# SamuelCancilla2/radar-point-cloud-tracking

Hardware: NVIDIA B200
Metric: fused_frames_per_s_through_stdbscan (higher is better)
Workload: dtype f32 (points) / f64 (neighbour test) / i32 (labels)

## Files before the change

### radar_point_cloud_tracking_b200/csrc/common.cuh

```cuda
#pragma once
#include <cuda_runtime.h>
#include <stdint.h>
#include <stdio.h>
#include <string.h>

#include <utility>
#include <vector>

#include "radarb200.h"

#define RB_WARP 32

struct rb_scratch {
    void* ptr = nullptr;
    size_t cap = 0;
};

enum rb_slot {
    RB_S_TILE_STATUS = 0,
    RB_S_SWEEP_FLAGS,
    RB_S_SPOKE_MASK,
    RB_S_REDUCE,
    RB_S_KEEP,
    RB_S_BLOCKSUM,
    RB_S_BLOCKSUM2,
    RB_S_CELL_ID,
    RB_S_CELL_START,
    RB_S_CELL_FILL,
    RB_S_SORT_IDX,
    RB_S_SX, RB_S_SY, RB_S_SZ, RB_S_ST,
    RB_S_CORE,
    RB_S_PARENT,
    RB_S_MINORIG,
    RB_S_FLAGS,
    RB_S_RANK,
    RB_S_SLABEL,
    RB_S_STATS,
    RB_S_MISC,
    RB_S_FUSE_GRID,
    RB_S_COMP_KEY,
    RB_S_PIPE, RB_S_PIPE_EDGES, RB_S_PIPE_TIMES,
    RB_S_B_NCORE, RB_S_B_PARENT, RB_S_B_LABEL, RB_S_B_MINKEY, RB_S_CORE_START, RB_S_CB_LIST,
    RB_S_CSV,
    RB_S_CLUSTERS,
    RB_S_LAND_FLAG,
    RB_S_SHARD_IDS, RB_S_SHARD_LOCAL, RB_S_SHARD_KEYS,
    RB_S_GROUP_TMP,
    RB_S_LAND_ORDERED,
    RB_S_REC_FRAMES,
    RB_S_REC_LOCAL,
    RB_S_REC_KEYS,
    RB_S_REC_KEYS_BIG,
    RB_S_REC_TABLE,
    RB_S_REC_CORE,
    RB_S_COUNT
};

struct rb_db_plan;
struct rb_comm;

struct rb_ctx {
    int device = 0;
    int sm_count = 0;
    int cc_major = 0, cc_minor = 0;
    int64_t l2_bytes = 0;
    int64_t launches = 0;
    rb_scratch slots[RB_S_COUNT];
    std::vector<void*> retired;
    void* pinned = nullptr;
    size_t pinned_cap = 0;
    rb_dbscan_stats last_stats;
    rb_db_plan* db_plan = nullptr;
    rb_comm* comm = nullptr;
    int64_t rec_key_cap = 0;
    int opt_dbscan_mode = 0;
    int opt_spoke_mask_variant = 0;
    int spoke_last_variant = 0;
    int opt_spoke_profile = 0;
    int opt_spoke_ring = 2;
    int opt_spoke_l2_hint = 1;
    int opt_mask_priority = 1;
    int prio_high = 0;
    int opt_mask_gate = 1;
    int opt_carveout = -1;
    unsigned attr_spoke_mask = 0;
    bool attr_land = false;
    cudaEvent_t spoke_ev[4] = {nullptr, nullptr, nullptr, nullptr};
};

void rb_set_error(const char* fmt, ...);
void rb_db_plan_free(rb_ctx* ctx);
void rb_comm_free(rb_ctx* ctx);
int rb_scratch_get(rb_ctx* ctx, rb_slot slot, size_t bytes, void** out);

#define RB_CUDA(call)                                                                      \
    do {                                                                                   \
        cudaError_t _e = (call);                                                           \
        if (_e != cudaSuccess) {                                                           \
            rb_set_error("%s:%d: %s -> %s", __FILE__, __LINE__, #call, cudaGetErrorString(_e)); \
            return RB_ERR_CUDA;                                                            \
        }                                                                                  \
    } while (0)

#define RB_LAUNCH_CHECK(ctx)                                                               \
    do {                                                                                   \
        (ctx)->launches++;                                                                 \
        cudaError_t _e = cudaGetLastError();                                               \
        if (_e != cudaSuccess) {                                                           \
            rb_set_error("%s:%d: kernel launch -> %s", __FILE__, __LINE__, cudaGetErrorString(_e)); \
            return RB_ERR_CUDA;                                                            \
        }                                                                                  \
    } while (0)

#define RB_REQUIRE(cond, msg)                                                              \
    do {                                                                                   \
        if (!(cond)) {                                                                     \
            rb_set_error("%s:%d: %s", __FILE__, __LINE__, msg);                            \
            return RB_ERR_ARG;                                                             \
        }                                                                                  \
    } while (0)

#define RB_TRY(expr)                                                                       \
    do {                                                                                   \
        int _rc = (expr);                                                                  \
        if (_rc != RB_OK) return _rc;                                                      \
    } while (0)

static inline int64_t rb_div_up(int64_t a, int64_t b) { return (a + b - 1) / b; }
// ... 82 lines not shown
```

### radar_point_cloud_tracking_b200/csrc/context.cu

```cuda
#include <stdarg.h>
#include <stdlib.h>

#include "common.cuh"

static thread_local char g_err[512] = "";

void rb_set_error(const char* fmt, ...) {
    va_list ap;
    va_start(ap, fmt);
    vsnprintf(g_err, sizeof g_err, fmt, ap);
    va_end(ap);
}

extern "C" const char* rb_last_error(void) { return g_err; }
extern "C" int rb_version(void) { return 1; }

extern "C" int rb_create(int device, rb_ctx** out) {
    if (!out) { rb_set_error("rb_create: out is NULL"); return RB_ERR_ARG; }
    *out = nullptr;
    int n = 0;
    cudaError_t e = cudaGetDeviceCount(&n);
    if (e != cudaSuccess || n <= 0) {
        rb_set_error("rb_create: no CUDA device (%s); this library has no CPU fallback",
                     e == cudaSuccess ? "device count 0" : cudaGetErrorString(e));
        return RB_ERR_CUDA;
    }
    if (device < 0 || device >= n) { rb_set_error("rb_create: bad device %d of %d", device, n); return RB_ERR_ARG; }
    int prev = -1;
    RB_CUDA(cudaGetDevice(&prev));
    struct Restore { int d; ~Restore() { if (d >= 0) cudaSetDevice(d); } } restore{prev == device ? -1 : prev};
    RB_CUDA(cudaSetDevice(device));
    cudaDeviceProp prop;
    RB_CUDA(cudaGetDeviceProperties(&prop, device));
    if (prop.major < 10) {
        rb_set_error("rb_create: device %d is sm_%d%d; this build is sm_100a only", device, prop.major, prop.minor);
        return RB_ERR_CUDA;
    }
    rb_ctx* ctx = new rb_ctx();
    ctx->device = device;
    ctx->sm_count = prop.multiProcessorCount;
    ctx->cc_major = prop.major;
    ctx->cc_minor = prop.minor;
    ctx->l2_bytes = prop.l2CacheSize;
    int prio_low = 0, prio_high = 0;
    if (cudaDeviceGetStreamPriorityRange(&prio_low, &prio_high) == cudaSuccess) ctx->prio_high = prio_high;
    memset(&ctx->last_stats, 0, sizeof ctx->last_stats);
    ctx->pinned_cap = 1 << 20;
    e = cudaMallocHost(&ctx->pinned, ctx->pinned_cap);
    if (e != cudaSuccess) {
        rb_set_error("rb_create: cudaMallocHost -> %s", cudaGetErrorString(e));
        delete ctx;
        return RB_ERR_NOMEM;
    }
    static const char* const env_opts[] = {"carveout", "spoke_ring", "spoke_l2_hint", "dbscan_mode", "spoke_mask_variant", "mask_gate", "mask_priority"};
    for (const char* name : env_opts) {
        char var[64] = "RB_OPT_";
        size_t k = strlen(var);
        for (const char* c = name; *c && k + 1 < sizeof var; ++c) var[k++] = (char)(*c >= 'a' && *c <= 'z' ? *c - 32 : *c);
        var[k] = 0;
        const char* v = getenv(var);
        if (v && *v && rb_set_option(ctx, name, atoll(v)) != RB_OK) { rb_destroy(ctx); return RB_ERR_ARG; }
    }
    *out = ctx;
    return RB_OK;
}

extern "C" void rb_destroy(rb_ctx* ctx) {
    if (!ctx) return;
    cudaSetDevice(ctx->device);
    for (int i = 0; i < RB_S_COUNT; ++i)
        if (ctx->slots[i].ptr) cudaFree(ctx->slots[i].ptr);
    for (void* p : ctx->retired) cudaFree(p);
    if (ctx->pinned) cudaFreeHost(ctx->pinned);
    for (int i = 0; i < 4; ++i)
        if (ctx->spoke_ev[i]) cudaEventDestroy(ctx->spoke_ev[i]);
    rb_db_plan_free(ctx);
    rb_comm_free(ctx);
    delete ctx;
}

extern "C" int rb_device_info(rb_ctx* ctx, int* sm_count, int* cc_major, int* cc_minor, int64_t* l2_bytes) {
    RB_REQUIRE(ctx, "ctx is NULL");
    if (sm_count) *sm_count = ctx->sm_count;
    if (cc_major) *cc_major = ctx->cc_major;
    if (cc_minor) *cc_minor = ctx->cc_minor;
    if (l2_bytes) *l2_bytes = ctx->l2_bytes;
    return RB_OK;
}

extern "C" int rb_set_option(rb_ctx* ctx, const char* name, int64_t value) {
    RB_REQUIRE(ctx && name, "NULL argument");
    if (!strcmp(name, "spoke_profile")) { ctx->opt_spoke_profile = value != 0; return RB_OK; }
    if (!strcmp(name, "dbscan_mode")) {
        RB_REQUIRE(value >= 0 && value <= 2, "dbscan_mode: 0 = auto, 1 = general algorithm, 2 = require the tight-cell algorithm");
        ctx->opt_dbscan_mode = (int)value;
        return RB_OK;
    }
    if (!strcmp(name, "spoke_mask_variant")) {
        RB_REQUIRE(value >= 0 && value <= 2, "spoke_mask_variant: 0 = auto, 1 = register-staged, 2 = TMA-staged");
        ctx->opt_spoke_mask_variant = (int)value;
        return RB_OK;
    }
    if (!strcmp(name, "spoke_ring")) {
        RB_REQUIRE(value >= 0 && value <= 3, "spoke_ring: 0 = 64 KiB x 3, 1 = 32 KiB x 4, 2 = 32 KiB x 3 (default), 3 = 48 KiB x 2");
        ctx->opt_spoke_ring = (int)value;
        return RB_OK;
    }
    if (!strcmp(name, "spoke_l2_hint")) { ctx->opt_spoke_l2_hint = value != 0; return RB_OK; }
    if (!strcmp(name, "mask_gate")) { ctx->opt_mask_gate = value != 0; return RB_OK; }
    if (!strcmp(name, "mask_priority")) { ctx->opt_mask_priority = value != 0; return RB_OK; }
    if (!strcmp(name, "carveout")) {
        RB_REQUIRE(value >= -1 && value <= 100, "carveout: -1 = the driver's choice per kernel, 0..100 = percent of the SM's shared memory");
        ctx->opt_carveout = (int)value;
        return RB_OK;
    }
    rb_set_error("rb_set_option: unknown option '%s'", name);
    return RB_ERR_ARG;
}

extern "C" int64_t rb_get_info(rb_ctx* ctx, const char* name) {
    if (!ctx || !name) return -1;
    if (!strcmp(name, "launches")) return ctx->launches;
    if (!strcmp(name, "spoke_profile")) return ctx->opt_spoke_profile;
    if (!strcmp(name, "spoke_mask_variant")) return ctx->opt_spoke_mask_variant;
    if (!strcmp(name, "dbscan_mode")) return ctx->opt_dbscan_mode;
    if (!strcmp(name, "spoke_last_variant")) return ctx->spoke_last_variant;
    if (!strcmp(name, "spoke_ring")) return ctx->opt_spoke_ring;
    if (!strcmp(name, "spoke_l2_hint")) return ctx->opt_spoke_l2_hint;
    if (!strcmp(name, "mask_gate")) return ctx->opt_mask_gate;
    if (!strcmp(name, "mask_priority")) return ctx->opt_mask_priority;
    if (!strcmp(name, "carveout")) return ctx->opt_carveout;
    int k = !strcmp(name, "spoke_mask_ns") ? 0 : !strcmp(name, "spoke_offsets_ns") ? 1 : !strcmp(name, "spoke_emit_ns") ? 2 : -1;
    if (k >= 0) {
        if (!ctx->spoke_ev[3]) return -1;
        if (cudaEventSynchronize(ctx->spoke_ev[3]) != cudaSuccess) return -1;
        float ms = 0.f;
        if (cudaEventElapsedTime(&ms, ctx->spoke_ev[k], ctx->spoke_ev[k + 1]) != cudaSuccess) return -1;
        return (int64_t)((double)ms * 1e6);
    }
    return -1;
}

extern "C" int64_t rb_launch_count(rb_ctx* ctx) { return ctx ? ctx->launches : -1; }

extern "C" int rb_trim(rb_ctx* ctx) {
    RB_REQUIRE(ctx, "ctx is NULL");
    for (void* p : ctx->retired) cudaFree(p);
    ctx->retired.clear();
    return RB_OK;
}

int rb_scratch_get(rb_ctx* ctx, rb_slot slot, size_t bytes, void** out) {
    rb_scratch& s = ctx->slots[slot];
    if (bytes == 0) bytes = 16;
    if (s.cap < bytes) {
        if (s.ptr) {
            ctx->retired.push_back(s.ptr);
            s.ptr = nullptr;
            s.cap = 0;
        }
        size_t want = bytes + bytes / 2;
        want = (want + 255) & ~size_t(255);
        cudaError_t e = cudaMalloc(&s.ptr, want);
        if (e != cudaSuccess) {
            rb_set_error("scratch slot %d: cudaMalloc(%zu) -> %s", (int)slot, want, cudaGetErrorString(e));
            s.ptr = nullptr;
            return RB_ERR_NOMEM;
        }
        s.cap = want;
    }
    *out = s.ptr;
    return RB_OK;
}

constexpr int SCAN_THREADS = 256;
constexpr int SCAN_ITEMS = 8;
constexpr int SCAN_TILE = SCAN_THREADS * SCAN_ITEMS;

// ... 102 lines not shown
```

### radar_point_cloud_tracking_b200/csrc/dbscan.cu

```cuda
#include <float.h>
#include <math.h>

#include "common.cuh"

namespace {

constexpr int DB_THREADS = 256;
constexpr long long KEY_NONE = 0x7fffffffffffffffLL;

struct DbGrid {
    double lo[3];
    double inv_cell;
    double tmin;
    double inv_wt;
    int n[3];
    int nt;
    int tr;
    int dim;
    int R;
    int tight;
};

struct DbPoints {
    const float* x; const float* y; const float* z;
// ... 299 lines not shown
__global__ void __launch_bounds__(DB_THREADS) dbg_keyout_kernel(int n, const uint8_t* __restrict__ core, const int* __restrict__ parent,
                                                               const int* __restrict__ sidx, const long long* __restrict__ minkey,
                                                               long long* __restrict__ comp_key) {
    int p = blockIdx.x * blockDim.x + threadIdx.x;
    if (p >= n) return;
    comp_key[sidx[p]] = core[p] == 1 ? minkey[parent[p]] : -1;
}

template <int DIM, bool WF>
__global__ void __launch_bounds__(DB_THREADS) dbg_border_kernel(Sorted s, DbGrid g, double eps2, float eps_t,
                                                               const uint8_t* __restrict__ core, const int* __restrict__ slabel,
                                                               const int* __restrict__ sidx, const long long* __restrict__ comp_key,
                                                               const int* __restrict__ open_list, const int* __restrict__ n_open,
                                                               int32_t* __restrict__ labels, unsigned long long* __restrict__ ctr) {
    const int total = *n_open;
    unsigned long long tests = 0;
    for (int i = blockIdx.x * blockDim.x + threadIdx.x; i < total; i += gridDim.x * blockDim.x) {
        const int p = open_list[i];
        Pt<DIM> a = load_pt<DIM>(s, p);
        int best = INT_MAX;
        for_each_candidate<DIM>(g, s.cell_start, s.cell[p], [&](int q) {
            if (core[q] == 1) {
                int lq = slabel[q];
                if (lq < best) {
                    if (WF) {
                        const int oq = sidx[q];
                        const long long start = comp_key[oq];
                        if (!(start < (long long)sidx[p] || start == (long long)oq)) return true;
                    }
                    ++tests;
                    if (is_neighbour<DIM>(a, load_pt<DIM>(s, q), eps2, eps_t)) best = lq;
                }
            }
            return best != 0;
        });
        if (best != INT_MAX) labels[sidx[p]] = best;
    }
    add_counter(ctr, tests);
}

struct Window {
    int x0, x1, y0, y1, z0, z1, t0, t1;
};
template <int DIM>
__device__ __forceinline__ Window window_of(const DbGrid& g, const CellPos& c) {
    Window w;
    w.x0 = max(c.cx - g.R, 0); w.x1 = min(c.cx + g.R, g.n[0] - 1);
    w.y0 = DIM > 1 ? max(c.cy - g.R, 0) : 0; w.y1 = DIM > 1 ? min(c.cy + g.R, g.n[1] - 1) : 0;
    w.z0 = DIM > 2 ? max(c.cz - g.R, 0) : 0; w.z1 = DIM > 2 ? min(c.cz + g.R, g.n[2] - 1) : 0;
    w.t0 = max(c.tb - g.tr, 0); w.t1 = min(c.tb + g.tr, g.nt - 1);
    return w;
}

template <int DIM, bool WF>
__global__ void __launch_bounds__(DB_THREADS) dbt_count_kernel(Sorted s, DbGrid g, int n, double eps2, int min_samples, int min_frames,
                                                              uint8_t* __restrict__ core, unsigned long long* __restrict__ ctr) {
    int p = blockIdx.x * blockDim.x + threadIdx.x;
    unsigned long long tests = 0;
    if (p < n) {
        const int cell = s.cell[p];
        const CellPos c = decode_cell(g, cell);
        const Window w = window_of<DIM>(g, c);
        const int per_t = g.n[0] * g.n[1] * g.n[2];
        const int sp = cell - c.tb * per_t;
        int cnt = 0;
        unsigned long long frames = 0;
        for (int tt = w.t0; tt <= w.t1; ++tt) {
            const int k = s.cell_start[tt * per_t + sp + 1] - s.cell_start[tt * per_t + sp];
            cnt += k;
            if (WF && k > 0) frames |= 1ull << (tt - w.t0);
        }
        auto open = [&]() { return cnt < min_samples || (WF && __popcll(frames) < min_frames); };
        if (open()) {
            const Pt<DIM> a = load_pt<DIM>(s, p);
            for (int tt = w.t0; tt <= w.t1 && open(); ++tt)
                for (int zz = w.z0; zz <= w.z1 && open(); ++zz)
                    for (int yy = w.y0; yy <= w.y1 && open(); ++yy) {
                        const int row = ((tt * g.n[2] + zz) * g.n[1] + yy) * g.n[0];
                        const bool own_row = zz == c.cz && yy == c.cy;
                        const int b = s.cell_start[row + w.x0], e = s.cell_start[row + w.x1 + 1];
                        int hb = e, he = e;
                        if (own_row) { hb = s.cell_start[row + c.cx]; he = s.cell_start[row + c.cx + 1]; }
                        for (int q = b; q < hb && open(); ++q) {
                            ++tests;
                            if (near_enough<DIM>(a, load_pt<DIM>(s, q), eps2)) { ++cnt; if (WF) frames |= 1ull << (tt - w.t0); }
                        }
                        for (int q = he; q < e && open(); ++q) {
                            ++tests;
                            if (near_enough<DIM>(a, load_pt<DIM>(s, q), eps2)) { ++cnt; if (WF) frames |= 1ull << (tt - w.t0); }
                        }
                    }
        }
        core[p] = !open() ? 1 : (cnt <= 1 ? 2 : 0);
    }
    add_counter(ctr, tests);
}

__global__ void __launch_bounds__(DB_THREADS) dbt_bucket_init_kernel(int64_t n_cells, int* __restrict__ b_ncore, int* __restrict__ b_parent,
                                                                    long long* __restrict__ b_minkey, int* __restrict__ n_cb) {
    int64_t b = (int64_t)blockIdx.x * blockDim.x + threadIdx.x;
    if (b == 0) *n_cb = 0;
    if (b < n_cells) { b_ncore[b] = 0; b_minkey[b] = KEY_NONE; }
    if (b == n_cells) b_ncore[b] = 0;
}

template <typename T, typename Op>
__device__ __forceinline__ T seg_reduce_sorted(T v, int key, Op op) {
    const unsigned lane = rb_lane();
#pragma unroll
    for (int d = 1; d < 32; d <<= 1) {
        const T ov = __shfl_down_sync(0xffffffffu, v, d);
        const int ok = __shfl_down_sync(0xffffffffu, key, d);
        if (lane + d < 32 && ok == key) v = op(v, ov);
    }
    return v;
}
__device__ __forceinline__ bool seg_head(int key) {
    const int prev = __shfl_up_sync(0xffffffffu, key, 1);
    return rb_lane() == 0 || prev != key;
}

__global__ void __launch_bounds__(DB_THREADS) dbt_bucket_stats_kernel(int n, const uint8_t* __restrict__ core, const int* __restrict__ scell,
                                                                     const int* __restrict__ sidx, const long long* __restrict__ gidx,
                                                                     int* __restrict__ b_ncore, long long* __restrict__ b_minkey) {
    const int p = blockIdx.x * blockDim.x + threadIdx.x;
    const bool is_core = p < n && core[p] == 1;
    const int b = p < n ? scell[p] : -1;
    const int cnt = seg_reduce_sorted<int>(is_core ? 1 : 0, b, [](int a, int c) { return a + c; });
    const long long key = seg_reduce_sorted<long long>(is_core ? point_key(gidx, sidx[p]) : KEY_NONE, b,
                                                       [](long long a, long long c) { return a < c ? a : c; });
    if (seg_head(b) && cnt > 0) {
        atomicAdd(b_ncore + b, cnt);
        atomicMin(b_minkey + b, key);
    }
}
// ... 306 lines not shown
            }
        }
    }
    add_counter(ctr, tests);
}

__global__ void __launch_bounds__(DB_THREADS) dbt_compmin_kernel(const int* __restrict__ cb_list, const int* __restrict__ n_cb,
                                                                int* __restrict__ b_parent, long long* __restrict__ b_minkey) {
    const int total = *n_cb;
    for (int i = blockIdx.x * blockDim.x + threadIdx.x; i < total; i += gridDim.x * blockDim.x) {
        const int b = cb_list[i];
        const int r = uf_find_ro(b_parent, b);
        if (r != b) {
            b_parent[b] = r;
            const long long k = b_minkey[b];
            if (k < *(volatile long long*)(b_minkey + r)) atomicMin(b_minkey + r, k);
        }
    }
}

__global__ void __launch_bounds__(DB_THREADS) dbt_keyout_kernel(int n, const uint8_t* __restrict__ core, const int* __restrict__ scell,
                                                               const int* __restrict__ sidx, const int* __restrict__ b_parent,
                                                               const long long* __restrict__ b_minkey, long long* __restrict__ comp_key) {
    int p = blockIdx.x * blockDim.x + threadIdx.x;
    if (p >= n) return;
    long long k = -1;
    if (core[p] == 1) { const int b = scell[p]; k = b_minkey[b_parent[b]]; }
    comp_key[sidx[p]] = k;
}

__global__ void __launch_bounds__(DB_THREADS) db_gather_labels_kernel(int n, const uint8_t* __restrict__ core, const int* __restrict__ sidx,
                                                                     const int* __restrict__ scell, const int32_t* core_label,
                                                                     int* __restrict__ slabel, int* __restrict__ b_label, int32_t* labels,
                                                                     int* __restrict__ open_list, int* __restrict__ n_open) {
    int p = blockIdx.x * blockDim.x + threadIdx.x;
    bool open = false;
    if (p < n) {
        const int orig = sidx[p];
        int lab = -1;
        if (core[p] == 1) { lab = core_label[orig]; if (b_label) b_label[scell[p]] = lab; }
        slabel[p] = lab;
        labels[orig] = lab;
        open = core[p] == 0;
    }
    const unsigned m = __ballot_sync(0xffffffffu, open);
    if (m) {
        int base = 0;
        if (rb_lane() == (unsigned)(__ffs(m) - 1)) base = atomicAdd(n_open, __popc(m));
        base = __shfl_sync(0xffffffffu, base, __ffs(m) - 1);
        if (open) open_list[base + __popc(m & rb_lanemask_lt())] = p;
    }
}

template <int DIM, bool WF>
__global__ void __launch_bounds__(DB_THREADS) dbt_border_kernel(Sorted s, DbGrid g, double eps2, const uint8_t* __restrict__ core,
                                                               const int* __restrict__ sidx, const int* __restrict__ open_list,
                                                               const int* __restrict__ n_open, const int* __restrict__ b_ncore,
                                                               const int* __restrict__ core_start, const int* __restrict__ b_label,
                                                               const int* __restrict__ b_parent, const long long* __restrict__ b_minkey,
                                                               int32_t* __restrict__ labels, unsigned long long* __restrict__ ctr) {
    const int total = *n_open;
    const int per_t = g.n[0] * g.n[1] * g.n[2];
    unsigned long long tests = 0;
    for (int k = blockIdx.x * blockDim.x + threadIdx.x; k < total; k += gridDim.x * blockDim.x) {
        const int p = open_list[k];
        const int cell = s.cell[p];
        const CellPos c = decode_cell(g, cell);
        const Window w = window_of<DIM>(g, c);
        const int sp = cell - c.tb * per_t;
        const long long me = sidx[p];
        int best = INT_MAX;
        for (int tt = w.t0; tt <= w.t1; ++tt) {
            const int b = tt * per_t + sp;
            if (b_ncore[b] <= 0) continue;
            if (WF) {
                const long long start = b_minkey[b_parent[b]];
                bool ok = start < me;
                for (int q = s.cell_start[b]; !ok && q < s.cell_start[b + 1]; ++q) ok = core[q] == 1 && (long long)sidx[q] == start;
                if (!ok) continue;
            }
            best = min(best, b_label[b]);
        }
        if (best != 0) {
            const Pt<DIM> a = load_pt<DIM>(s, p);
            for (int tt = w.t0; tt <= w.t1 && best != 0; ++tt)
                for (int zz = w.z0; zz <= w.z1 && best != 0; ++zz)
                    for (int yy = w.y0; yy <= w.y1 && best != 0; ++yy) {
                        const int row = ((tt * g.n[2] + zz) * g.n[1] + yy) * g.n[0];
                        if (core_start[row + w.x1 + 1] == core_start[row + w.x0]) continue;
                        for (int xx = w.x0; xx <= w.x1; ++xx) {
                            const int b = row + xx;
                            if (b_ncore[b] == 0 || (xx == c.cx && yy == c.cy && zz == c.cz)) continue;
                            const int lb = b_label[b];
                            if (lb >= best) continue;
                            const long long start = WF ? b_minkey[b_parent[b]] : 0;
                            const bool any_core = !WF || start < me;
                            for (int q = s.cell_start[b]; q < s.cell_start[b + 1]; ++q) {
                                if (core[q] != 1 || (!any_core && (long long)sidx[q] != start)) continue;
                                ++tests;
                                if (near_enough<DIM>(a, load_pt<DIM>(s, q), eps2)) { best = lb; break; }
                            }
                        }
                    }
        }
        if (best != INT_MAX) labels[me] = best;
    }
    add_counter(ctr, tests);
}

__global__ void __launch_bounds__(DB_THREADS) db_core_out_kernel(int n, const uint8_t* __restrict__ core, const int* __restrict__ sidx,
                                                                uint8_t* __restrict__ core_out) {
    int p = blockIdx.x * blockDim.x + threadIdx.x;
    if (p < n) core_out[sidx[p]] = core[p] == 1;
}

__global__ void __launch_bounds__(DB_THREADS) db_core_in_kernel(int n, const uint8_t* __restrict__ core_in, const int* __restrict__ sidx,
                                                               uint8_t* __restrict__ core) {
    int p = blockIdx.x * blockDim.x + threadIdx.x;
    if (p < n) core[p] = core_in[sidx[p]] ? 1 : (core[p] == 2 ? 2 : 0);
}

__global__ void __launch_bounds__(DB_THREADS) db_rootflag_kernel(int n, const long long* __restrict__ comp_key, int* __restrict__ flags) {
    int i = blockIdx.x * blockDim.x + threadIdx.x;
    if (i < n) flags[i] = comp_key[i] == (long long)i;
}

__global__ void __launch_bounds__(DB_THREADS) db_rank_labels_kernel(int n, const long long* __restrict__ comp_key, const int* __restrict__ rank,
                                                                   int32_t* __restrict__ labels) {
    int i = blockIdx.x * blockDim.x + threadIdx.x;
    if (i >= n) return;
    const long long k = comp_key[i];
    labels[i] = k >= 0 ? rank[k] : -1;
}

__global__ void __launch_bounds__(DB_THREADS) db_relabel_kernel(int64_t n, const long long* __restrict__ keys, const long long* __restrict__ table_keys,
                                                               const int32_t* __restrict__ table_ids, int64_t m, int32_t* __restrict__ out) {
    int64_t i = (int64_t)blockIdx.x * blockDim.x + threadIdx.x;
    if (i >= n) return;
    const long long k = keys[i];
    int32_t id = -1;
    if (k >= 0 && m > 0) {
        int64_t lo = 0, hi = m;
        while (lo < hi) { int64_t mid = (lo + hi) >> 1; if (table_keys[mid] < k) lo = mid + 1; else hi = mid; }
        if (lo < m && table_keys[lo] == k) id = table_ids[lo];
    }
    out[i] = id;
}

template <typename T>
int scratch(rb_ctx* ctx, rb_slot slot, size_t count, T** out) {
    void* p;
    int rc = rb_scratch_get(ctx, slot, sizeof(T) * count, &p);
    *out = (T*)p;
// ... 143 lines not shown
        RB_CUDA(cudaMemcpyAsync(h, P.d_misc, sizeof(int) * 9, cudaMemcpyDeviceToHost, stream));
        RB_CUDA(cudaStreamSynchronize(stream));
        for (int k = 0; k < 4; ++k) { mn[k] = ord2f(h[k]); mx[k] = ord2f(h[4 + k]); }
        times_integer = h[8] == 0;
    }

    RB_TRY(choose_grid(mn, mx, times_integer, DIM, n64, eps_space, eps_time, ctx->opt_dbscan_mode, &P.g, &P.cell, &P.wt));
    const DbGrid& g = P.g;
    P.n_cells = (int64_t)g.n[0] * g.n[1] * g.n[2] * g.nt;

    int *cell_id, *slot;
    RB_TRY(scratch(ctx, RB_S_CELL_ID, (size_t)n, &cell_id));
    RB_TRY(scratch(ctx, RB_S_CELL_FILL, (size_t)n, &slot));
    RB_TRY(scratch(ctx, RB_S_CELL_START, (size_t)P.n_cells + 1, &P.cell_start));
    RB_TRY(scratch(ctx, RB_S_SORT_IDX, (size_t)n * 2, &P.sidx));
    P.scell = P.sidx + n;
    RB_TRY(scratch(ctx, RB_S_SX, (size_t)n, &P.sx));
    RB_TRY(scratch(ctx, RB_S_SY, (size_t)n, &P.sy));
    RB_TRY(scratch(ctx, RB_S_SZ, (size_t)n, &P.sz));
    RB_TRY(scratch(ctx, RB_S_ST, (size_t)n, &P.st));
    RB_TRY(scratch(ctx, RB_S_CORE, (size_t)n, &P.core));
    RB_TRY(scratch(ctx, RB_S_PARENT, (size_t)n, &P.parent));
    RB_TRY(scratch(ctx, RB_S_MINORIG, (size_t)n, &P.minkey));
    RB_TRY(scratch(ctx, RB_S_FLAGS, (size_t)n + 1, &P.flags));
    RB_TRY(scratch(ctx, RB_S_RANK, (size_t)n + 1, &P.rank));
    RB_TRY(scratch(ctx, RB_S_SLABEL, (size_t)n, &P.slabel));
    RB_TRY(scratch(ctx, RB_S_COMP_KEY, (size_t)n, &P.comp_key));
    if (g.tight) {
        RB_TRY(scratch(ctx, RB_S_B_NCORE, (size_t)P.n_cells + 1, &P.b_ncore));
        RB_TRY(scratch(ctx, RB_S_B_PARENT, (size_t)P.n_cells, &P.b_parent));
        RB_TRY(scratch(ctx, RB_S_B_LABEL, (size_t)P.n_cells, &P.b_label));
        RB_TRY(scratch(ctx, RB_S_B_MINKEY, (size_t)P.n_cells, &P.b_minkey));
        RB_TRY(scratch(ctx, RB_S_CORE_START, (size_t)P.n_cells + 1, &P.core_start));
        RB_TRY(scratch(ctx, RB_S_CB_LIST, (size_t)(P.n_cells < n ? P.n_cells : n) * 7 + 8, &P.cb_list));
        P.cb_bbox = P.cb_list + (size_t)(P.n_cells < n ? P.n_cells : n) + 1;
        P.cb_slot = P.b_label;
    }
    RB_CUDA(cudaMemsetAsync(P.cell_start, 0, sizeof(int) * ((size_t)P.n_cells + 1), stream));
    RB_CUDA(rb_launch(ctx, db_cell_kernel, dim3(blocks), dim3(DB_THREADS), 0, stream, pts, g, n64, cell_id, slot, P.cell_start, hint ? (int*)(P.d_ctr + 4) : nullptr));
    RB_LAUNCH_CHECK(ctx);
    RB_TRY(rb_exclusive_scan_i32(ctx, P.cell_start, P.cell_start, P.n_cells + 1, nullptr, stream));
    RB_CUDA(rb_launch(ctx, db_scatter_kernel, dim3(blocks), dim3(DB_THREADS), 0, stream, pts, DIM, n64, cell_id, slot, P.cell_start, P.sidx, P.scell, P.sx, P.sy, P.sz,
                                                        P.st));
    RB_LAUNCH_CHECK(ctx);
    P.valid = true;
    return RB_OK;
}

template <int DIM>
int phase_cores(rb_ctx* ctx, rb_db_plan& P, cudaStream_t stream) {
    const unsigned blocks = (unsigned)rb_div_up(P.n, DB_THREADS);
    const Sorted s = sorted_view(P);
    const bool wf = P.min_frames > 0;
    if (P.g.tight && wf) RB_CUDA(rb_launch(ctx, dbt_count_kernel<DIM, true>, dim3(blocks), dim3(DB_THREADS), 0, stream, s, P.g, P.n, P.eps2, P.min_samples, P.min_frames, P.core, P.d_ctr + 0));
    else if (P.g.tight) RB_CUDA(rb_launch(ctx, dbt_count_kernel<DIM, false>, dim3(blocks), dim3(DB_THREADS), 0, stream, s, P.g, P.n, P.eps2, P.min_samples, 0, P.core, P.d_ctr + 0));
    else if (wf) RB_CUDA(rb_launch(ctx, dbg_count_kernel<DIM, true>, dim3(blocks), dim3(DB_THREADS), 0, stream, s, P.g, P.n, P.eps2, P.eps_t, P.min_samples, P.min_frames, P.core, P.d_ctr + 0));
    else RB_CUDA(rb_launch(ctx, dbg_count_kernel<DIM, false>, dim3(blocks), dim3(DB_THREADS), 0, stream, s, P.g, P.n, P.eps2, P.eps_t, P.min_samples, 0, P.core, P.d_ctr + 0));
    RB_LAUNCH_CHECK(ctx);
    P.have_cores = true;
    P.have_components = false;
    return RB_OK;
}

template <int DIM>
int phase_components(rb_ctx* ctx, rb_db_plan& P, const long long* gidx, cudaStream_t stream) {
    const int n = P.n;
    const unsigned blocks = (unsigned)rb_div_up(n, DB_THREADS);
    const Sorted s = sorted_view(P);
    if (P.g.tight) {
        const unsigned cblocks = (unsigned)rb_div_up(P.n_cells + 1, DB_THREADS);
        RB_CUDA(rb_launch(ctx, dbt_bucket_init_kernel, dim3(cblocks), dim3(DB_THREADS), 0, stream, P.n_cells, P.b_ncore, P.b_parent, P.b_minkey, P.d_ncb));
        RB_LAUNCH_CHECK(ctx);
        RB_CUDA(rb_launch(ctx, dbt_bucket_stats_kernel, dim3(blocks), dim3(DB_THREADS), 0, stream, n, P.core, P.scell, P.sidx, gidx, P.b_ncore, P.b_minkey));
        RB_LAUNCH_CHECK(ctx);
        const unsigned lblocks = (unsigned)rb_div_up(P.n_cells, (int64_t)DB_THREADS * LIST_PER_THREAD);
        RB_CUDA(rb_launch(ctx, dbt_bucket_list_kernel, dim3(lblocks), dim3(DB_THREADS), 0, stream, P.n_cells, P.b_ncore, P.cb_list, P.d_ncb, P.cb_slot, P.cb_bbox, P.b_parent));
        RB_LAUNCH_CHECK(ctx);
        RB_CUDA(rb_launch(ctx, dbt_bucket_bbox_kernel<DIM>, dim3(blocks), dim3(DB_THREADS), 0, stream, s, n, P.core, P.cb_slot, P.cb_bbox));
        RB_LAUNCH_CHECK(ctx);
        RB_TRY(rb_exclusive_scan_i32(ctx, P.b_ncore, P.core_start, P.n_cells + 1, nullptr, stream));
        const int64_t max_buckets = P.n_cells < n ? P.n_cells : n;
        const int64_t want = rb_div_up(max_buckets, DB_THREADS);
        const unsigned ublocks = (unsigned)(want < (int64_t)ctx->sm_count * 16 ? (want > 0 ? want : 1) : (int64_t)ctx->sm_count * 16);
        const int64_t want2 = rb_div_up(max_buckets, DB_THREADS);
        const unsigned mblocks = (unsigned)(want2 < (int64_t)ctx->sm_count * 8 ? (want2 > 0 ? want2 : 1) : (int64_t)ctx->sm_count * 8);
        RB_CUDA(rb_launch(ctx, dbt_link_time_kernel, dim3(mblocks), dim3(DB_THREADS), 0, stream, P.g, P.cb_list, P.d_ncb, P.b_ncore, P.b_parent));
        RB_LAUNCH_CHECK(ctx);
        RB_CUDA(rb_launch(ctx, dbt_flatten_kernel, dim3(mblocks), dim3(DB_THREADS), 0, stream, P.cb_list, P.d_ncb, P.b_parent));
        RB_LAUNCH_CHECK(ctx);
        RB_CUDA(rb_launch(ctx, dbt_union_kernel<DIM>, dim3(ublocks), dim3(DB_THREADS), 0, stream, s, P.g, P.cb_list, P.d_ncb, P.core, P.b_ncore, P.b_parent, P.cb_slot,
                                                                  P.cb_bbox, P.eps2, P.d_ctr + 1));
        RB_LAUNCH_CHECK(ctx);
        RB_CUDA(rb_launch(ctx, dbt_compmin_kernel, dim3(mblocks), dim3(DB_THREADS), 0, stream, P.cb_list, P.d_ncb, P.b_parent, P.b_minkey));
        RB_LAUNCH_CHECK(ctx);
        RB_CUDA(rb_launch(ctx, dbt_keyout_kernel, dim3(blocks), dim3(DB_THREADS), 0, stream, n, P.core, P.scell, P.sidx, P.b_parent, P.b_minkey, P.comp_key));
        RB_LAUNCH_CHECK(ctx);
    } else {
        RB_CUDA(rb_launch(ctx, dbg_init_kernel, dim3(blocks), dim3(DB_THREADS), 0, stream, n, P.parent, P.minkey));
        RB_LAUNCH_CHECK(ctx);
        RB_CUDA(rb_launch(ctx, dbg_union_kernel<DIM>, dim3(blocks), dim3(DB_THREADS), 0, stream, s, P.g, n, P.eps2, P.eps_t, P.core, P.parent, P.d_ctr + 1));
        RB_LAUNCH_CHECK(ctx);
        RB_CUDA(rb_launch(ctx, dbg_minkey_kernel, dim3(blocks), dim3(DB_THREADS), 0, stream, n, P.core, P.parent, P.sidx, gidx, P.minkey));
        RB_LAUNCH_CHECK(ctx);
        RB_CUDA(rb_launch(ctx, dbg_keyout_kernel, dim3(blocks), dim3(DB_THREADS), 0, stream, n, P.core, P.parent, P.sidx, P.minkey, P.comp_key));
        RB_LAUNCH_CHECK(ctx);
    }
    P.have_components = true;
    return RB_OK;
}

template <int DIM>
int phase_assign(rb_ctx* ctx, rb_db_plan& P, const int32_t* core_label, int32_t* labels, cudaStream_t stream) {
    const int n = P.n;
    const unsigned blocks = (unsigned)rb_div_up(n, DB_THREADS);
    const Sorted s = sorted_view(P);
    int* open_list = P.rank;
    int* n_open = P.d_misc + 34;
    RB_CUDA(cudaMemsetAsync(n_open, 0, sizeof(int), stream));
    RB_CUDA(rb_launch(ctx, db_gather_labels_kernel, dim3(blocks), dim3(DB_THREADS), 0, stream, n, P.core, P.sidx, P.scell, core_label, P.slabel,
                      P.g.tight ? P.b_label : nullptr, labels, open_list, n_open));
    RB_LAUNCH_CHECK(ctx);
    const bool wf = P.min_frames > 0;
    const unsigned wblocks = (unsigned)(blocks < (unsigned)ctx->sm_count * 8 ? blocks : (unsigned)ctx->sm_count * 8);
    if (P.g.tight && wf)
        RB_CUDA(rb_launch(ctx, dbt_border_kernel<DIM, true>, dim3(wblocks), dim3(DB_THREADS), 0, stream, s, P.g, P.eps2, P.core, P.sidx, open_list, n_open,
                          P.b_ncore, P.core_start, P.b_label, P.b_parent, P.b_minkey, labels, P.d_ctr + 2));
    else if (P.g.tight)
        RB_CUDA(rb_launch(ctx, dbt_border_kernel<DIM, false>, dim3(wblocks), dim3(DB_THREADS), 0, stream, s, P.g, P.eps2, P.core, P.sidx, open_list, n_open,
                          P.b_ncore, P.core_start, P.b_label, P.b_parent, P.b_minkey, labels, P.d_ctr + 2));
    else if (wf)
        RB_CUDA(rb_launch(ctx, dbg_border_kernel<DIM, true>, dim3(wblocks), dim3(DB_THREADS), 0, stream, s, P.g, P.eps2, P.eps_t, P.core, P.slabel, P.sidx,
                          P.comp_key, open_list, n_open, labels, P.d_ctr + 2));
    else
        RB_CUDA(rb_launch(ctx, dbg_border_kernel<DIM, false>, dim3(wblocks), dim3(DB_THREADS), 0, stream, s, P.g, P.eps2, P.eps_t, P.core, P.slabel, P.sidx,
                          P.comp_key, open_list, n_open, labels, P.d_ctr + 2));
    RB_LAUNCH_CHECK(ctx);
    return RB_OK;
}

#define DB_DISPATCH(P, call)                                  \
    ((P).dim == 3 ? call<3> : (P).dim == 2 ? call<2> : call<1>)

int fetch_stats(rb_ctx* ctx, rb_db_plan& P, int64_t* n_clusters, cudaStream_t stream) {
    unsigned long long* hc = (unsigned long long*)ctx->pinned;
    RB_CUDA(cudaMemcpyAsync(hc, P.d_ctr, sizeof(unsigned long long) * 5, cudaMemcpyDeviceToHost, stream));
    RB_CUDA(cudaStreamSynchronize(stream));
    if (hc[4] != 0) {
        rb_set_error("ST-DBSCAN: the hinted box does not contain every point / time (rb_stdbscan_hint); the result is invalid");
        return RB_ERR_ARG;
    }
    rb_dbscan_stats& stt = ctx->last_stats;
    memset(&stt, 0, sizeof stt);
    stt.n_points = P.n;
    stt.n_cells = P.n_cells;
    stt.n_clusters = (int64_t)(int)(hc[3] & 0xffffffffu);
    stt.n_core = -1;
    stt.pair_tests_count = (int64_t)hc[0];
    stt.pair_tests_union = (int64_t)hc[1];
    stt.pair_tests_border = (int64_t)hc[2];
    stt.cell_size = P.cell;
    stt.time_bin = P.wt;
    stt.dims[0] = P.g.n[0]; stt.dims[1] = P.g.n[1]; stt.dims[2] = P.g.n[2]; stt.dims[3] = P.g.nt;
    stt.time_radius = P.g.tr;
    stt.tight = P.g.tight;
    if (n_clusters) *n_clusters = stt.n_clusters;
    return RB_OK;
}

}

int rb_stdbscan_plan_hinted(rb_ctx* ctx, const float* x, const float* y, const float* z, int64_t stride,
                            const float* times, int64_t n, double eps_space, float eps_time, int min_samples,
                            const rb_stdbscan_hint* hint, void* stream_);

extern "C" int rb_stdbscan_plan(rb_ctx* ctx, const float* x, const float* y, const float* z, int64_t stride,
                                const float* times, int64_t n, double eps_space, float eps_time, int min_samples,
                                void* stream_) {
    return rb_stdbscan_plan_hinted(ctx, x, y, z, stride, times, n, eps_space, eps_time, min_samples, nullptr, stream_);
}

extern "C" int rb_stdbscan_plan_hinted(rb_ctx* ctx, const float* x, const float* y, const float* z, int64_t stride,
                                       const float* times, int64_t n, double eps_space, float eps_time, int min_samples,
                                       const rb_stdbscan_hint* hint, void* stream_) {
// ... 154 lines not shown
```

Before: 200,700.

## Trim tight-window DBSCAN scans to reachable cells and count fully-inside cells wholesale

Adds a per-point reachability mask that works out which rows and x-ranges of the 5x5x5 cell window can actually hold neighbours within eps. The count and border kernels skip unreachable rows and narrow the x span, which cuts memory loads and distance tests. Cells that lie entirely inside the eps ball are added to the count as a whole, or taken as a border hit without per-point tests. The price is extra per-thread register and arithmetic work, plus reliance on conservative float error margins for correctness.

```diff
diff --git a/radar_point_cloud_tracking_b200/csrc/common.cuh b/radar_point_cloud_tracking_b200/csrc/common.cuh
--- a/radar_point_cloud_tracking_b200/csrc/common.cuh
+++ b/radar_point_cloud_tracking_b200/csrc/common.cuh
@@ -74,6 +74,7 @@
     rb_comm* comm = nullptr;
     int64_t rec_key_cap = 0;
     int opt_dbscan_mode = 0;
+    int opt_dbscan_trim = 1;
     int opt_spoke_mask_variant = 0;
     int spoke_last_variant = 0;
     int opt_spoke_profile = 0;
diff --git a/radar_point_cloud_tracking_b200/csrc/context.cu b/radar_point_cloud_tracking_b200/csrc/context.cu
--- a/radar_point_cloud_tracking_b200/csrc/context.cu
+++ b/radar_point_cloud_tracking_b200/csrc/context.cu
@@ -52,7 +52,7 @@
         delete ctx;
         return RB_ERR_NOMEM;
     }
-    static const char* const env_opts[] = {"carveout", "spoke_ring", "spoke_l2_hint", "dbscan_mode", "spoke_mask_variant", "mask_gate", "mask_priority"};
+    static const char* const env_opts[] = {"carveout", "spoke_ring", "spoke_l2_hint", "dbscan_mode", "dbscan_trim", "spoke_mask_variant", "mask_gate", "mask_priority"};
     for (const char* name : env_opts) {
         char var[64] = "RB_OPT_";
         size_t k = strlen(var);
@@ -96,6 +96,11 @@
         ctx->opt_dbscan_mode = (int)value;
         return RB_OK;
     }
+    if (!strcmp(name, "dbscan_trim")) {
+        RB_REQUIRE(value == 0 || value == 1, "dbscan_trim: 1 = visit only the reachable cells of the tight window (default), 0 = the whole window");
+        ctx->opt_dbscan_trim = (int)value;
+        return RB_OK;
+    }
     if (!strcmp(name, "spoke_mask_variant")) {
         RB_REQUIRE(value >= 0 && value <= 2, "spoke_mask_variant: 0 = auto, 1 = register-staged, 2 = TMA-staged");
         ctx->opt_spoke_mask_variant = (int)value;
@@ -124,6 +129,7 @@
     if (!strcmp(name, "spoke_profile")) return ctx->opt_spoke_profile;
     if (!strcmp(name, "spoke_mask_variant")) return ctx->opt_spoke_mask_variant;
     if (!strcmp(name, "dbscan_mode")) return ctx->opt_dbscan_mode;
+    if (!strcmp(name, "dbscan_trim")) return ctx->opt_dbscan_trim;
     if (!strcmp(name, "spoke_last_variant")) return ctx->spoke_last_variant;
     if (!strcmp(name, "spoke_ring")) return ctx->opt_spoke_ring;
     if (!strcmp(name, "spoke_l2_hint")) return ctx->opt_spoke_l2_hint;
diff --git a/radar_point_cloud_tracking_b200/csrc/dbscan.cu b/radar_point_cloud_tracking_b200/csrc/dbscan.cu
--- a/radar_point_cloud_tracking_b200/csrc/dbscan.cu
+++ b/radar_point_cloud_tracking_b200/csrc/dbscan.cu
@@ -375,7 +375,79 @@
     return w;
 }
 
-template <int DIM, bool WF>
+constexpr unsigned REACH_ROW = 1u << 4, REACH_IN0 = 1u << 5, REACH_INL = 1u << 6, REACH_INH = 1u << 7;
+constexpr unsigned REACH_FULL = REACH_ROW | 2u | 2u << 2;
+
+template <int DIM>
+struct Reach { unsigned long long slab[DIM > 2 ? 5 : 1]; };
+
+template <int DIM>
+__host__ __device__ __forceinline__ Reach<DIM> reach_of(const DbGrid& g, const Pt<DIM>& a, const CellPos& c, double eps2) {
+    constexpr int RY = DIM > 1 ? 2 : 0, RZ = DIM > 2 ? 2 : 0;
+    Reach<DIM> r;
+    const double T = eps2 * g.inv_cell * g.inv_cell;
+    const float t_out = (float)(T * (1.0 + 1e-5)), t_in = (float)(T * (1.0 - 1e-5));
+    const float v[3] = {a.x, a.y, a.z};
+    const int ck[3] = {c.cx, c.cy, c.cz};
+    float sf[3] = {0.f, 0.f, 0.f}, sg[3] = {0.f, 0.f, 0.f};
+    bool lo_edge[3] = {false, false, false}, hi_edge[3] = {false, false, false};
+    bool c_edge[3] = {false, false, false};
+#pragma unroll
+    for (int k = 0; k < DIM; ++k) {
+        const double u = ((double)v[k] - g.lo[k]) * g.inv_cell;
+        const double sd = u - (double)ck[k];
+        sf[k] = (float)sd;
+        sg[k] = (float)(1e-15 * (fabs(u) + (double)ck[k] + 4.0)) + 2.4e-7f * (fabsf(sf[k]) + 4.f);
+        c_edge[k] = !(ck[k] > 0 && ck[k] < g.n[k] - 1);
+        lo_edge[k] = !(ck[k] - 1 > 0 && ck[k] - 1 < g.n[k] - 1);
+        hi_edge[k] = !(ck[k] + 1 > 0 && ck[k] + 1 < g.n[k] - 1);
+    }
+    auto gap2 = [&](int k, int d) {
+        const float gp = fmaxf((d > 0 ? (float)d - sf[k] : sf[k] - (float)(d + 1)) - sg[k], 0.f);
+        return gp * gp;
+    };
+    auto far2 = [&](int k, int d) {
+        const bool edge = d < 0 ? lo_edge[k] : d > 0 ? hi_edge[k] : c_edge[k];
+        const float f = fmaxf((float)(d + 1) - sf[k], sf[k] - (float)d) + sg[k];
+        return edge ? INFINITY : f * f;
+    };
+    const float gxm1 = gap2(0, -1), gxm2 = gap2(0, -2), gxp1 = gap2(0, 1), gxp2 = gap2(0, 2);
+    const float fxm1 = far2(0, -1), fx0 = far2(0, 0), fxp1 = far2(0, 1);
+#pragma unroll
+    for (int dz = -RZ; dz <= RZ; ++dz) {
+        unsigned long long slab = 0;
+#pragma unroll
+        for (int dy = -RY; dy <= RY; ++dy) {
+            const float g_yz = (dy ? gap2(1, dy) : 0.f) + (dz ? gap2(2, dz) : 0.f);
+            unsigned b = 0;
+            if (!(g_yz > t_out)) {
+                b = REACH_ROW;
+                b |= (unsigned)(gxm1 + g_yz <= t_out) + (unsigned)(gxm2 + g_yz <= t_out);
+                b |= ((unsigned)(gxp1 + g_yz <= t_out) + (unsigned)(gxp2 + g_yz <= t_out)) << 2;
+                if (abs(dy) <= 1 && abs(dz) <= 1) {
+                    const float f_yz = (DIM > 1 ? far2(1, dy) : 0.f) + (DIM > 2 ? far2(2, dz) : 0.f);
+                    if (fx0 + f_yz < t_in) b |= REACH_IN0;
+                    if (fxm1 + f_yz < t_in) b |= REACH_INL;
+                    if (fxp1 + f_yz < t_in) b |= REACH_INH;
+                }
+            }
+            slab |= (unsigned long long)b << (8 * (dy + RY));
+        }
+        r.slab[dz + RZ] = slab;
+    }
+    return r;
+}
+
+template <int DIM>
+__host__ __device__ __forceinline__ unsigned reach_row(const Reach<DIM>& r, int dy, int dz) {
+    constexpr int RY = DIM > 1 ? 2 : 0, RZ = DIM > 2 ? 2 : 0;
+    unsigned long long slab = r.slab[0];
+#pragma unroll
+    for (int k = 1; k < (DIM > 2 ? 5 : 1); ++k) slab = dz + RZ == k ? r.slab[k] : slab;
+    return (unsigned)(slab >> (8 * (dy + RY))) & 0xffu;
+}
+
+template <int DIM, bool WF, bool TRIM>
 __global__ void __launch_bounds__(DB_THREADS) dbt_count_kernel(Sorted s, DbGrid g, int n, double eps2, int min_samples, int min_frames,
                                                               uint8_t* __restrict__ core, unsigned long long* __restrict__ ctr) {
     int p = blockIdx.x * blockDim.x + threadIdx.x;
@@ -396,14 +468,27 @@
         auto open = [&]() { return cnt < min_samples || (WF && __popcll(frames) < min_frames); };
         if (open()) {
             const Pt<DIM> a = load_pt<DIM>(s, p);
+            Reach<DIM> reach;
+            if (TRIM) reach = reach_of<DIM>(g, a, c, eps2);
             for (int tt = w.t0; tt <= w.t1 && open(); ++tt)
                 for (int zz = w.z0; zz <= w.z1 && open(); ++zz)
                     for (int yy = w.y0; yy <= w.y1 && open(); ++yy) {
+                        const unsigned r = TRIM ? reach_row<DIM>(reach, yy - c.cy, zz - c.cz) : REACH_FULL;
+                        if (!(r & REACH_ROW)) continue;
                         const int row = ((tt * g.n[2] + zz) * g.n[1] + yy) * g.n[0];
                         const bool own_row = zz == c.cz && yy == c.cy;
-                        const int b = s.cell_start[row + w.x0], e = s.cell_start[row + w.x1 + 1];
+                        const int xa = max(c.cx - (int)(r & 3u), 0), xb = min(c.cx + (int)(r >> 2 & 3u), g.n[0] - 1);
+                        const int b = s.cell_start[row + xa], e = s.cell_start[row + xb + 1];
                         int hb = e, he = e;
-                        if (own_row) { hb = s.cell_start[row + c.cx]; he = s.cell_start[row + c.cx + 1]; }
+                        if (own_row || (r & REACH_IN0)) {
+                            hb = s.cell_start[row + c.cx - (int)(r >> 6 & 1u)];
+                            he = s.cell_start[row + c.cx + 1 + (int)(r >> 7 & 1u)];
+                            int whole = he - hb;
+                            if (own_row)
+                                whole = (r & (REACH_INL | REACH_INH)) ? whole - (s.cell_start[row + c.cx + 1] - s.cell_start[row + c.cx]) : 0;
+                            cnt += whole;
+                            if (WF && whole > 0) frames |= 1ull << (tt - w.t0);
+                        }
                         for (int q = b; q < hb && open(); ++q) {
                             ++tests;
                             if (near_enough<DIM>(a, load_pt<DIM>(s, q), eps2)) { ++cnt; if (WF) frames |= 1ull << (tt - w.t0); }
@@ -816,7 +901,7 @@
     }
 }
 
-template <int DIM, bool WF>
+template <int DIM, bool WF, bool TRIM>
 __global__ void __launch_bounds__(DB_THREADS) dbt_border_kernel(Sorted s, DbGrid g, double eps2, const uint8_t* __restrict__ core,
                                                                const int* __restrict__ sidx, const int* __restrict__ open_list,
                                                                const int* __restrict__ n_open, const int* __restrict__ b_ncore,
@@ -847,22 +932,34 @@
         }
         if (best != 0) {
             const Pt<DIM> a = load_pt<DIM>(s, p);
+            Reach<DIM> reach;
+            if (TRIM) reach = reach_of<DIM>(g, a, c, eps2);
             for (int tt = w.t0; tt <= w.t1 && best != 0; ++tt)
                 for (int zz = w.z0; zz <= w.z1 && best != 0; ++zz)
                     for (int yy = w.y0; yy <= w.y1 && best != 0; ++yy) {
+                        const unsigned r = TRIM ? reach_row<DIM>(reach, yy - c.cy, zz - c.cz) : REACH_FULL;
+                        if (!(r & REACH_ROW)) continue;
+                        const int xa = max(c.cx - (int)(r & 3u), 0), xb = min(c.cx + (int)(r >> 2 & 3u), g.n[0] - 1);
                         const int row = ((tt * g.n[2] + zz) * g.n[1] + yy) * g.n[0];
-                        if (core_start[row + w.x1 + 1] == core_start[row + w.x0]) continue;
-                        for (int xx = w.x0; xx <= w.x1; ++xx) {
+                        if (core_start[row + xb + 1] == core_start[row + xa]) continue;
+                        for (int xx = xa; xx <= xb; ++xx) {
                             const int b = row + xx;
                             if (b_ncore[b] == 0 || (xx == c.cx && yy == c.cy && zz == c.cz)) continue;
                             const int lb = b_label[b];
                             if (lb >= best) continue;
                             const long long start = WF ? b_minkey[b_parent[b]] : 0;
                             const bool any_core = !WF || start < me;
+                            const unsigned in_bit = xx == c.cx ? REACH_IN0 : xx < c.cx ? REACH_INL : REACH_INH;
+                            const bool whole = (r & in_bit) && xx >= c.cx - 1 && xx <= c.cx + 1;
+                            if (whole && any_core) { best = lb; continue; }
                             for (int q = s.cell_start[b]; q < s.cell_start[b + 1]; ++q) {
                                 if (core[q] != 1 || (!any_core && (long long)sidx[q] != start)) continue;
-                                ++tests;
-                                if (near_enough<DIM>(a, load_pt<DIM>(s, q), eps2)) { best = lb; break; }
+                                if (!whole) {
+                                    ++tests;
+                                    if (!near_enough<DIM>(a, load_pt<DIM>(s, q), eps2)) continue;
+                                }
+                                best = lb;
+                                break;
                             }
                         }
                     }
@@ -1112,9 +1209,12 @@
     const unsigned blocks = (unsigned)rb_div_up(P.n, DB_THREADS);
     const Sorted s = sorted_view(P);
     const bool wf = P.min_frames > 0;
-    if (P.g.tight && wf) RB_CUDA(rb_launch(ctx, dbt_count_kernel<DIM, true>, dim3(blocks), dim3(DB_THREADS), 0, stream, s, P.g, P.n, P.eps2, P.min_samples, P.min_frames, P.core, P.d_ctr + 0));
-    else if (P.g.tight) RB_CUDA(rb_launch(ctx, dbt_count_kernel<DIM, false>, dim3(blocks), dim3(DB_THREADS), 0, stream, s, P.g, P.n, P.eps2, P.min_samples, 0, P.core, P.d_ctr + 0));
-    else if (wf) RB_CUDA(rb_launch(ctx, dbg_count_kernel<DIM, true>, dim3(blocks), dim3(DB_THREADS), 0, stream, s, P.g, P.n, P.eps2, P.eps_t, P.min_samples, P.min_frames, P.core, P.d_ctr + 0));
+    const bool trim = ctx->opt_dbscan_trim != 0;
+    if (P.g.tight) {
+        auto kernel = wf ? (trim ? dbt_count_kernel<DIM, true, true> : dbt_count_kernel<DIM, true, false>)
+                         : (trim ? dbt_count_kernel<DIM, false, true> : dbt_count_kernel<DIM, false, false>);
+        RB_CUDA(rb_launch(ctx, kernel, dim3(blocks), dim3(DB_THREADS), 0, stream, s, P.g, P.n, P.eps2, P.min_samples, wf ? P.min_frames : 0, P.core, P.d_ctr + 0));
+    } else if (wf) RB_CUDA(rb_launch(ctx, dbg_count_kernel<DIM, true>, dim3(blocks), dim3(DB_THREADS), 0, stream, s, P.g, P.n, P.eps2, P.eps_t, P.min_samples, P.min_frames, P.core, P.d_ctr + 0));
     else RB_CUDA(rb_launch(ctx, dbg_count_kernel<DIM, false>, dim3(blocks), dim3(DB_THREADS), 0, stream, s, P.g, P.n, P.eps2, P.eps_t, P.min_samples, 0, P.core, P.d_ctr + 0));
     RB_LAUNCH_CHECK(ctx);
     P.have_cores = true;
@@ -1182,13 +1282,13 @@
     RB_LAUNCH_CHECK(ctx);
     const bool wf = P.min_frames > 0;
     const unsigned wblocks = (unsigned)(blocks < (unsigned)ctx->sm_count * 8 ? blocks : (unsigned)ctx->sm_count * 8);
-    if (P.g.tight && wf)
-        RB_CUDA(rb_launch(ctx, dbt_border_kernel<DIM, true>, dim3(wblocks), dim3(DB_THREADS), 0, stream, s, P.g, P.eps2, P.core, P.sidx, open_list, n_open,
+    const bool trim = ctx->opt_dbscan_trim != 0;
+    if (P.g.tight) {
+        auto kernel = wf ? (trim ? dbt_border_kernel<DIM, true, true> : dbt_border_kernel<DIM, true, false>)
+                         : (trim ? dbt_border_kernel<DIM, false, true> : dbt_border_kernel<DIM, false, false>);
+        RB_CUDA(rb_launch(ctx, kernel, dim3(wblocks), dim3(DB_THREADS), 0, stream, s, P.g, P.eps2, P.core, P.sidx, open_list, n_open,
                           P.b_ncore, P.core_start, P.b_label, P.b_parent, P.b_minkey, labels, P.d_ctr + 2));
-    else if (P.g.tight)
-        RB_CUDA(rb_launch(ctx, dbt_border_kernel<DIM, false>, dim3(wblocks), dim3(DB_THREADS), 0, stream, s, P.g, P.eps2, P.core, P.sidx, open_list, n_open,
-                          P.b_ncore, P.core_start, P.b_label, P.b_parent, P.b_minkey, labels, P.d_ctr + 2));
-    else if (wf)
+    } else if (wf)
         RB_CUDA(rb_launch(ctx, dbg_border_kernel<DIM, true>, dim3(wblocks), dim3(DB_THREADS), 0, stream, s, P.g, P.eps2, P.eps_t, P.core, P.slabel, P.sidx,
                           P.comp_key, open_list, n_open, labels, P.d_ctr + 2));
     else
```

New measurement: 200,700, median of 6. No clear change (+0.0%).
